# tgialoimtr/cnn_lstm_ctc_ocr

Measured on AMD Instinct MI355X. Metric: line-crops/sec (train step) at 32x256 bs=256; CER vs ref, higher is better.
Workload: dtype bf16

## Files before the change

cnn_lstm_ctc_ocr_amd/csrc/common.h:

```cpp
#pragma once
#include <hip/hip_runtime.h>
#include <cstdint>
#include <cstddef>
#include <mutex>
#include "ocrk.h"

typedef __bf16 bf16;

namespace ocrk {

void set_error(const char* fmt, ...);
int launch_status(const char* what);

inline hipStream_t as_stream(void* s) { return reinterpret_cast<hipStream_t>(s); }

inline int64_t cdiv(int64_t a, int64_t b) { return (a + b - 1) / b; }

constexpr int kMaxDevices = 64;
constexpr int kMaxCuWords = 32;
inline int current_device() {
    int d = 0;
    (void)hipGetDevice(&d);
    return d < 0 ? 0 : (d >= kMaxDevices ? kMaxDevices - 1 : d);
}
// ... 26 lines not shown
    OPT_CONV_ROWS,
    OPT_CONV_ROWS_WIDE,
    OPT_CONV_WGRAD_BLOCKS,
    OPT_LSTM_SPIN_LIMIT,
    OPT_PERSIST_LATE,
    OPT_LSTM_BWD_KSPLIT,
    OPT_LSTM_BWD_PB16,
    OPT_LSTM_BWD_R16,
    OPT_CTC_LDS,
    OPT_PP_PERSIST_NK,
    OPT_PP_DEEP,
    OPT_NT_F32_EXACT,
    OPT_NT_F32_MASK,
    OPT_NT_F32_X6,
    OPT_BEAM_WAVE,
    OPT_BN_BWD_BLOCKS,
    OPT_BN_ROUTE,
    OPT_BN_ROUTE_SEG,
    OPT_BN_ROUTE_NCH,
    OPT_CONV_TN_ITEMS,
    OPT_CONV_TN4_ITEMS,
    OPT_CONV_WGRAD_CUS,
    OPT_F32_MFMA,
    OPT_GEMM_NT,
    OPT_GEMM_NT_STAGED,
    OPT_GEMM_PP,
    OPT_GEMM_PPTN,
    OPT_PP_MIN_N,
    OPT_GEMM_TN,
    OPT_LSTM_DMA,
    OPT_LSTM_BWD_DMA,
    OPT_LSTM_FWD_R16,
    OPT_NT_TAP_UNIFORM,
    OPT_COUNT
};
int64_t opt(Option o);

}

#define OCRK_REQUIRE(cond, ...)                       \
    do {                                                \
        if (!(cond)) {                                  \
            ocrk::set_error(__VA_ARGS__);               \
            return OCRK_ERR_INVALID_ARG;                \
        }                                               \
    } while (0)

__device__ __forceinline__ float to_f32(float x) { return x; }
__device__ __forceinline__ float to_f32(bf16 x) { return (float)x; }
template <typename T> __device__ __forceinline__ T from_f32(float x);
template <> __device__ __forceinline__ float from_f32<float>(float x) { return x; }
template <> __device__ __forceinline__ bf16 from_f32<bf16>(float x) { return (bf16)x; }

__device__ __forceinline__ float sigmoidf_(float x) { return 1.0f / (1.0f + expf(-x)); }

struct F8 { float v[8]; };

template <typename T> __device__ __forceinline__ F8 load8(const T* p);
template <> __device__ __forceinline__ F8 load8<float>(const float* p) {
    F8 r;
    float4 a = reinterpret_cast<const float4*>(p)[0], b = reinterpret_cast<const float4*>(p)[1];
    r.v[0] = a.x; r.v[1] = a.y; r.v[2] = a.z; r.v[3] = a.w;
    r.v[4] = b.x; r.v[5] = b.y; r.v[6] = b.z; r.v[7] = b.w;
    return r;
}
template <> __device__ __forceinline__ F8 load8<bf16>(const bf16* p) {
    union { uint4 q; bf16 e[8]; } u;
    u.q = *reinterpret_cast<const uint4*>(p);
    F8 r;
// ... 94 lines not shown
```

cnn_lstm_ctc_ocr_amd/csrc/gemm.h:

```cpp
#pragma once
#include "common.h"

namespace ocrk {

enum AMode { A_ROWK = 0, A_COLK = 1, A_IM2COL = 2, A_IM2COL_FLIP = 3, A_IM2COL_T = 4 };
enum BMode { B_NK = 0, B_KN = 1 };

struct GemmParams {
    int M, N, K;
    int batch;
    const void* A; int64_t lda; int64_t strideA;
    const void* B; int64_t ldb; int64_t strideB;
    void* C; int64_t ldc; int64_t strideC;
    int c_bf16;
    const float* bias; int64_t strideBias;
    const void* mask; int64_t ldmask;
    int accumulate;
    int relu;
    float alpha;
    float* stats;
    float* splitk_ws;
    int splits;
    int k_chunk;
    int convH, convW, convC;
    int epi_staged;
    const void* mask_bits;
    void* relu_bits;
};

struct TileIdx { int bm, bn; bool valid; };
__device__ __forceinline__ TileIdx xcd_tile(int tm, int tn) {
    const int nT = tm * tn, per = (nT + 7) >> 3;
    const int t = (int)(blockIdx.x & 7) * per + (int)(blockIdx.x >> 3);
    if (t >= nT) return {0, 0, false};
    constexpr int GM = 4;
    const int gsz = GM * tn, grp = t / gsz, first = grp * GM;
    const int gm = min(GM, tm - first), w = t - grp * gsz;
    return {first + w % gm, w / gm, true};
}
__host__ __forceinline__ unsigned xcd_grid(int tm, int tn) { return 8u * (unsigned)((tm * tn + 7) / 8); }

int gemm(const GemmParams& p, int amode, int bmode, int dtype, hipStream_t stream);

size_t gemm_splitk_ws_bytes(int M, int N, int batch, int splits);
int splitk_finish(const GemmParams& p, hipStream_t stream);

int gemm_nt(const GemmParams& p, int amode, int bmode, int dtype, hipStream_t stream);
bool f32_exact_mfma();

int gemm_pp(const GemmParams& p, int amode, int bmode, int dtype, hipStream_t stream);

bool gemm_pptn_covers(int amode, int M, int N, int convC);
int gemm_pptn(const GemmParams& p, int amode, int bmode, int dtype, hipStream_t stream);

int gemm_tn(const GemmParams& p, int amode, int bmode, int dtype, hipStream_t stream);

}
```

cnn_lstm_ctc_ocr_amd/csrc/gemm.hip:

```cpp
#include <atomic>
#include <cstdlib>
#include <type_traits>

#include "gemm.h"
#include "mfma_util.h"

namespace ocrk {

template <int AM, typename CT>
__device__ __forceinline__ const CT* a_addr(const GemmParams& p, const CT* A, int m, int k, bool& ok) {
    if constexpr (AM == A_ROWK) {
        ok = m < p.M && k < p.K;
        return A + (int64_t)m * p.lda + k;
    } else if constexpr (AM == A_COLK) {
        ok = m < p.M && k < p.K;
        return A + (int64_t)k * p.lda + m;
    } else {
        int pix, kidx;
        if constexpr (AM == A_IM2COL_T) { pix = k; kidx = m; ok = k < p.K && m < p.M; }
        else { pix = m; kidx = k; ok = m < p.M && k < p.K; }
        const int C = p.convC, W = p.convW, H = p.convH;
        int tap = kidx / C, c = kidx - tap * C;
        int kh = tap / 3, kw = tap - kh * 3;
        int w = pix % W, t2 = pix / W, h = t2 % H, b = t2 / H;
// ... 498 lines not shown
}

template <typename CT>
static int dispatch_modes(const GemmParams& p, int amode, int bmode, hipStream_t s) {
#define GM(AMx, BMx) if (amode == AMx && bmode == BMx) return launch_tiles<CT, AMx, BMx>(p, s)
    GM(A_ROWK, B_NK);
    GM(A_ROWK, B_KN);
    GM(A_COLK, B_KN);
    GM(A_IM2COL, B_NK);
    GM(A_IM2COL_FLIP, B_NK);
    GM(A_IM2COL_T, B_KN);
#undef GM
    set_error("gemm: unsupported operand modes A=%d B=%d", amode, bmode);
    return OCRK_ERR_INVALID_ARG;
}

int gemm(const GemmParams& p, int amode, int bmode, int dtype, hipStream_t stream) {
    if (p.M <= 0 || p.N <= 0 || p.batch <= 0) return OCRK_OK;
    OCRK_REQUIRE(p.K >= 0 && p.splits >= 1 && p.k_chunk > 0 && p.k_chunk % 32 == 0,
                 "gemm: bad K=%d splits=%d k_chunk=%d", p.K, p.splits, p.k_chunk);
    bool a_rows = (amode == A_COLK || amode == A_IM2COL_T);
    OCRK_REQUIRE(p.K % 8 == 0 || (a_rows && bmode == B_KN),
                 "gemm: K=%d must be a multiple of 8 for k-contiguous operands", p.K);
    OCRK_REQUIRE(!a_rows || p.M % 8 == 0, "gemm: M=%d must be a multiple of 8 for this A mode", p.M);
    OCRK_REQUIRE(bmode != B_KN || p.N % 8 == 0, "gemm: N=%d must be a multiple of 8 for B_KN", p.N);
    OCRK_REQUIRE(amode < A_IM2COL || p.convC % 8 == 0, "gemm: conv channels must be a multiple of 8");
    OCRK_REQUIRE(!(p.stats && (p.splits > 1 || p.batch > 1)), "gemm: stats need splits=1, batch=1");
    OCRK_REQUIRE(!(p.accumulate && p.c_bf16), "gemm: accumulate needs an f32 C");
    if (p.mask_bits || p.relu_bits) {
        const int st = gemm_nt(p, amode, bmode, dtype, stream);
        OCRK_REQUIRE(st >= 0, "gemm: ReLU bit masks need the NT engine (bf16 C, staged epilogue) for this shape");
        return st;
    }
    int nt = gemm_pp(p, amode, bmode, dtype, stream);
    if (nt >= 0) return nt != OCRK_OK ? nt : splitk_finish(p, stream);
    nt = gemm_nt(p, amode, bmode, dtype, stream);
    if (nt < 0) nt = gemm_pptn(p, amode, bmode, dtype, stream);
    if (nt < 0) nt = gemm_tn(p, amode, bmode, dtype, stream);
    if (nt >= 0) return nt != OCRK_OK ? nt : splitk_finish(p, stream);
    if (dtype == OCRK_BF16) return dispatch_modes<bf16>(p, amode, bmode, stream);
    if (dtype == OCRK_F32) return dispatch_modes<float>(p, amode, bmode, stream);
    set_error("gemm: unsupported dtype %d", dtype);
    return OCRK_ERR_INVALID_ARG;
}

}

extern "C" int ocrk_set_f32_gemm_mode(int mode) {
    OCRK_REQUIRE(mode == 0 || mode == 1, "ocrk_set_f32_gemm_mode: mode %d not 0 (bf16x3) or 1 (exact)", mode);
    return ocrk::g_f32_mode.exchange(mode);
}

extern "C" int ocrk_f32_gemm_exact(void) { return ocrk::f32_exact_mfma() ? 1 : 0; }

extern "C" size_t ocrk_gemm_workspace_size(int M, int N, int batch, int splits) {
    return ocrk::gemm_splitk_ws_bytes(M, N, batch, splits);
}

extern "C" int ocrk_gemm(int trans_a, int trans_b, int M, int N, int K, float alpha, const void* A,
                         int64_t lda, int64_t stride_a, const void* B, int64_t ldb, int64_t stride_b,
                         void* C, int64_t ldc, int64_t stride_c, int c_dtype, const float* bias,
                         int relu, int accumulate, int batch, int dtype, int splits, void* ws,
                         size_t ws_bytes, void* stream) {
    ocrk::GemmParams p = {};
    p.M = M; p.N = N; p.K = K; p.batch = batch < 1 ? 1 : batch;
    p.A = A; p.lda = lda; p.strideA = stride_a;
    p.B = B; p.ldb = ldb; p.strideB = stride_b;
    p.C = C; p.ldc = ldc; p.strideC = stride_c;
    p.c_bf16 = c_dtype == OCRK_BF16;
// ... 14 lines not shown
```

cnn_lstm_ctc_ocr_amd/csrc/gemm_pp.hip:

```cpp
#include "gemm.h"
#include "mfma_util.h"

namespace ocrk {

namespace {

constexpr unsigned PP_OOB = 0x80000000u;

__device__ __forceinline__ void pp_dma16(__amdgpu_buffer_rsrc_t r, void* lds, unsigned voff) {
    __builtin_amdgcn_raw_ptr_buffer_load_lds(r, (__attribute__((address_space(3))) void*)lds, 16, voff, 0, 0, 0);
}

__device__ __forceinline__ void pp_barrier() {
    asm volatile("" ::: "memory");
    __builtin_amdgcn_s_barrier();
    asm volatile("" ::: "memory");
}

template <int N> __device__ __forceinline__ void vm_wait_nop() {}

typedef unsigned short u16x4 __attribute__((ext_vector_type(4)));

struct PPItem { int m0, n0, zb, zs; };
__device__ __forceinline__ PPItem pp_item(int w, int tm, int tn, int splits, int BM, int BN) {
    const int nT = tm * tn;
    const int z = w / nT, t = w - z * nT;
    constexpr int GM = 4;
    const int gsz = GM * tn, grp = t / gsz, first = grp * GM;
    const int gm = min(GM, tm - first), r = t - grp * gsz;
    PPItem it;
    it.m0 = (first + r % gm) * BM;
    it.n0 = (r / gm) * BN;
    it.zb = z / splits;
    it.zs = z - it.zb * splits;
    return it;
}

template <int AM, int BN, bool STATS, bool MASK>
__global__ void __launch_bounds__(512) gemm_pp_kernel(const GemmParams p) {
    constexpr int BM = 256, BK = 64, ROWB = 128;
    constexpr int WCOLS = BN / 4;
    constexpr int QN = WCOLS / 32;
    constexpr int A_BYTES = BM * ROWB, BUF = (BM + BN) * ROWB;
    constexpr int NUA = 2;
    constexpr int NUB = BN / 128;
    constexpr int HBLK = WCOLS / 16;
    constexpr int NU0 = NUA, NU1 = NUB, NU2 = NUB, NU3 = NUA;
    constexpr int PITCH = WCOLS * 2 + 16, CPRW = WCOLS / 8;
    constexpr int CR = BN == 256 ? 32 : 64;
    constexpr int NST = 128 * CPRW / 64;
    static_assert(BN == 256 || BN == 128, "BN");
    static_assert(8 * CR * PITCH <= BUF, "staging fits the freed buffer");
    extern __shared__ __attribute__((aligned(16))) char smem[];
    const bf16* mask = reinterpret_cast<const bf16*>(p.mask);

    const int tid = threadIdx.x, lane = tid & 63;
    const int wave = __builtin_amdgcn_readfirstlane(tid >> 6);
    const int wm = wave >> 2, wn = wave & 3;
    const int i16 = lane & 15, g = lane >> 4, sw = lane & 7;

    const int tm = (p.M + BM - 1) / BM, tn = (p.N + BN - 1) / BN;
    const int nitems = tm * tn * p.batch * p.splits;
    const int per = (nitems + 7) >> 3;
    const int xcd = blockIdx.x & 7, slot = blockIdx.x >> 3, sp = gridDim.x >> 3;
    const int wend = min(nitems, (xcd + 1) * per);
    int w_issue = xcd * per + slot;
    if (w_issue >= wend) return;

    const int lrow = lane >> 3;
// ... 287 lines not shown
                    for (int j = 0; j < 2 * QN; ++j) {
                        u16x4 o;
#pragma unroll
                        for (int r = 0; r < 4; ++r)
                            o[r] = __builtin_bit_cast(unsigned short, (bf16)acc[h * (CR / 16) + i][j][r]);
                        *reinterpret_cast<u16x4*>(stg + (i * 16 + i16) * PITCH + (j * 16 + 4 * g) * 2) = o;
                    }
                __builtin_amdgcn_wave_barrier();
#pragma unroll
                for (int q = 0; q < CR * CPRW / 64; ++q) {
                    const int r = r0 + q * (64 / CPRW);
                    const int m = cur_it.m0 + wm * 128 + h * CR + r;
                    const u32x4 v = *reinterpret_cast<const u32x4*>(stg + r * PITCH + c8 * 16);
                    const unsigned off = (m < p.M && n < p.N) ? (unsigned)(((int64_t)m * p.ldc + n) * 2) : PP_OOB;
                    __builtin_amdgcn_raw_buffer_store_b128(v, rc, off, 0, 0);
                }
                __builtin_amdgcn_wave_barrier();
            }
        }
        asm volatile("s_waitcnt lgkmcnt(0)" ::: "memory");
        pp_barrier();
        w_comp += sp;
        if (w_comp >= wend) break;
        cur_it = pp_item(w_comp, tm, tn, p.splits, BM, BN);
        c_nk = max(1, (min(p.K, cur_it.zs * p.k_chunk + p.k_chunk) - cur_it.zs * p.k_chunk + BK - 1) / BK);
        c_kt = 0;
        after_epi = true;
#pragma unroll
        for (int i = 0; i < 8; ++i)
#pragma unroll
            for (int j = 0; j < 2 * QN; ++j) acc[i][j] = floatx4{0.f, 0.f, 0.f, 0.f};
        if (wm == 1) pp_barrier();
    }
}

__device__ __forceinline__ void vm_wait_n(int n) {
    n = __builtin_amdgcn_readfirstlane(n);
    n = n > 63 ? 63 : n;
    switch (n) {
#define VW1(i) case i: vm_wait<i>(); break;
#define VW8(b) VW1(b) VW1(b + 1) VW1(b + 2) VW1(b + 3) VW1(b + 4) VW1(b + 5) VW1(b + 6) VW1(b + 7)
        VW8(0) VW8(8) VW8(16) VW8(24) VW8(32) VW8(40) VW8(48) VW8(56)
#undef VW8
#undef VW1
    default: vm_wait<0>();
    }
}

template <int FAST>
__device__ __forceinline__ void vm_wait_fast(int n) {
    n = __builtin_amdgcn_readfirstlane(n);
    if (n == FAST) vm_wait<FAST>();
    else vm_wait_n(n);
}

template <int BN>
__global__ void __launch_bounds__(512) gemm_pp_deep_kernel(const GemmParams p) {
    constexpr int BM = 256, BK = 64, ROWB = 128;
    constexpr int WCOLS = BN / 4;
    constexpr int QN = WCOLS / 32;
    constexpr int A_BYTES = BM * ROWB, BUF = (BM + BN) * ROWB;
    constexpr int NUA = 2, NUB = BN / 128;
    constexpr int HBLK = WCOLS / 16;
    constexpr int PITCH = WCOLS * 2 + 16, CPRW = WCOLS / 8;
    constexpr int CR = 16;
    constexpr int NST = 128 * CPRW / 64;
    static_assert(BN == 256 || BN == 128, "BN");
    static_assert(CR * PITCH <= (BN == 256 ? 4096 : 2048), "a wave's staging fits its slot piece");
    extern __shared__ __attribute__((aligned(16))) char smem[];

    const int tid = threadIdx.x, lane = tid & 63;
    const int wave = __builtin_amdgcn_readfirstlane(tid >> 6);
    const int wm = wave >> 2, wn = wave & 3;
    const int i16 = lane & 15, g = lane >> 4, sw = lane & 7;

    const int tm = (p.M + BM - 1) / BM, tn = (p.N + BN - 1) / BN;
    const int nitems = tm * tn * p.batch * p.splits;
    const int per = (nitems + 7) >> 3;
    const int xcd = blockIdx.x & 7, slot = blockIdx.x >> 3, sp = gridDim.x >> 3;
    const int wend = min(nitems, (xcd + 1) * per);
    int w_issue = xcd * per + slot;
    if (w_issue >= wend) return;

    const int lrow = lane >> 3;
    const int cs = (lane & 7) ^ lrow;
    int arow[4];
// ... 319 lines not shown
```

cnn_lstm_ctc_ocr_amd/csrc/mfma_util.h:

```cpp
#pragma once
#include "common.h"

namespace ocrk {

typedef __bf16 bf16x8 __attribute__((ext_vector_type(8)));
typedef float floatx4 __attribute__((ext_vector_type(4)));

typedef unsigned int u32x4 __attribute__((ext_vector_type(4)));
typedef float f32x4 __attribute__((ext_vector_type(4)));

template <typename CT> struct V8;
template <> struct V8<bf16> {
    u32x4 q;
    __device__ __forceinline__ unsigned short e(int i) const {
        return (unsigned short)(q[i >> 1] >> (16 * (i & 1)));
    }
};
template <> struct V8<float> {
    f32x4 q0, q1;
    __device__ __forceinline__ float e(int i) const { return i < 4 ? q0[i] : q1[i - 4]; }
};
template <typename CT> struct RawT;
template <> struct RawT<bf16> { using T = unsigned short; };
template <> struct RawT<float> { using T = float; };
// ... 65 lines not shown
    split3_bf16(x.q0[0], x.q0[1], h[0], m[0], l[0]);
    split3_bf16(x.q0[2], x.q0[3], h[1], m[1], l[1]);
    split3_bf16(x.q1[0], x.q1[1], h[2], m[2], l[2]);
    split3_bf16(x.q1[2], x.q1[3], h[3], m[3], l[3]);
    hi = u32x4{h[0], h[1], h[2], h[3]};
    mid = u32x4{m[0], m[1], m[2], m[3]};
    lo = u32x4{l[0], l[1], l[2], l[3]};
}

__device__ __forceinline__ __amdgpu_buffer_rsrc_t uniform_rsrc(const void* base, int64_t bytes) {
    const uint64_t b = (uint64_t)base;
    const unsigned lo = __builtin_amdgcn_readfirstlane((unsigned)b);
    const unsigned hi = __builtin_amdgcn_readfirstlane((unsigned)(b >> 32));
    const int nb = __builtin_amdgcn_readfirstlane(bytes > 0x7fffffff ? 0x7fffffff : (int)bytes);
    return __builtin_amdgcn_make_buffer_rsrc((void*)(((uint64_t)hi << 32) | lo), 0, nb, 0x00020000);
}

typedef int i32x4_t __attribute__((ext_vector_type(4)));
__device__ __forceinline__ i32x4_t uniform_rsrc_words(const void* base, int64_t bytes) {
    const uint64_t b = (uint64_t)base;
    const int lo = (int)__builtin_amdgcn_readfirstlane((unsigned)b);
    const int hi = (int)__builtin_amdgcn_readfirstlane((unsigned)(b >> 32) & 0xffffu);
    const int nb = __builtin_amdgcn_readfirstlane(bytes > 0x7fffffff ? 0x7fffffff : (int)bytes);
    return i32x4_t{lo, hi, nb, 0x00020000};
}

__device__ __forceinline__ void lds_dma16_asm(const i32x4_t& r, void* lds, unsigned voff) {
    const unsigned a = __builtin_amdgcn_readfirstlane(
        (unsigned)(uintptr_t)(__attribute__((address_space(3))) char*)lds);
    asm volatile("s_nop 0\n\tbuffer_load_dwordx4 %0, %1, 0 offen lds"
                 :: "v"(voff), "s"(r), "{m0}"(a) : "memory");
}

}
```

cnn_lstm_ctc_ocr_amd/csrc/runtime.hip:

```cpp
#include <atomic>
#include <cstdarg>
#include <cstdlib>
#include <cstdio>
#include <cstring>
#include <mutex>
#include "common.h"

namespace ocrk {

static thread_local char g_err[1024] = "";

void set_error(const char* fmt, ...) {
    va_list ap;
    va_start(ap, fmt);
    vsnprintf(g_err, sizeof(g_err), fmt, ap);
    va_end(ap);
}

int launch_status(const char* what) {
    hipError_t e = hipGetLastError();
    if (e != hipSuccess) {
        set_error("%s: %s", what, hipGetErrorString(e));
        return OCRK_ERR_HIP;
    }
    return OCRK_OK;
}

namespace {
struct OptDef {
    const char* name;
    int64_t def;
    bool exp = false;
};
constexpr OptDef kOptDefs[OPT_COUNT] = {
    {"CONV_DIRECT", 1}, {"CONV_ROWS", 1}, {"CONV_ROWS_WIDE", 1}, {"CONV_WGRAD_BLOCKS", 1},
    {"LSTM_SPIN_LIMIT", 0}, {"PERSIST_LATE", 1}, {"LSTM_BWD_KSPLIT", 0, true}, {"LSTM_BWD_PB16", 0, true},
    {"LSTM_BWD_R16", 1}, {"CTC_LDS", 1}, {"PP_PERSIST_NK", 8}, {"PP_DEEP", 0, true}, {"NT_F32_EXACT", 1},
    {"NT_F32_MASK", 1},
    {"NT_F32_X6", 0}, {"BEAM_WAVE", 1}, {"BN_BWD_BLOCKS", 2048}, {"BN_ROUTE", 1}, {"BN_ROUTE_SEG", 8}, {"BN_ROUTE_NCH", 4},
    {"CONV_TN_ITEMS", 192},
    {"CONV_TN4_ITEMS", 512}, {"CONV_WGRAD_CUS", 192}, {"F32_MFMA", 0}, {"GEMM_NT", 1}, {"GEMM_NT_STAGED", 1},
    {"GEMM_PP", 1}, {"GEMM_PPTN", 1}, {"PP_MIN_N", 512}, {"GEMM_TN", 1}, {"LSTM_DMA", 1}, {"LSTM_BWD_DMA", 1},
    {"LSTM_FWD_R16", 1}, {"NT_TAP_UNIFORM", 1},
};
std::atomic<int64_t> g_opts[OPT_COUNT];
std::once_flag g_opts_once;

#ifdef OCRK_EXPERIMENTS
constexpr bool kExperiments = true;
#else
constexpr bool kExperiments = false;
#endif

void init_opts() {
    for (int i = 0; i < OPT_COUNT; ++i) {
        if (kOptDefs[i].exp && !kExperiments) {
            g_opts[i].store(kOptDefs[i].def, std::memory_order_relaxed);
            continue;
        }
        char env[64];
        snprintf(env, sizeof(env), "OCRK_%s", kOptDefs[i].name);
        const char* e = getenv(env);
        g_opts[i].store(e && *e ? atoll(e) : kOptDefs[i].def, std::memory_order_relaxed);
    }
}

int find_opt(const char* name) {
    if (!name) return -1;
    if (!strncmp(name, "OCRK_", 5)) name += 5;
    for (int i = 0; i < OPT_COUNT; ++i)
        if (!strcmp(name, kOptDefs[i].name)) return kOptDefs[i].exp && !kExperiments ? -1 : i;
    return -1;
}
}

int64_t opt(Option o) {
    std::call_once(g_opts_once, init_opts);
    return g_opts[o].load(std::memory_order_relaxed);
}

}

extern "C" {

int ocrk_version(void) { return OCRK_ABI_VERSION; }

int ocrk_set_option(const char* name, int64_t value, int64_t* prev) {
    const int i = ocrk::find_opt(name);
    OCRK_REQUIRE(i >= 0, "ocrk_set_option: unknown option '%s'", name ? name : "(null)");
    ocrk::opt((ocrk::Option)i);
    const int64_t old = ocrk::g_opts[i].exchange(value, std::memory_order_relaxed);
    if (prev) *prev = old;
    return OCRK_OK;
}

int ocrk_get_option(const char* name, int64_t* value) {
    const int i = ocrk::find_opt(name);
    OCRK_REQUIRE(i >= 0 && value, "ocrk_get_option: unknown option '%s' or null slot", name ? name : "(null)");
    *value = ocrk::opt((ocrk::Option)i);
    return OCRK_OK;
}

const char* ocrk_last_error(void) { return ocrk::g_err; }

int ocrk_timer_create(void** ev) {
    OCRK_REQUIRE(ev != nullptr, "ocrk_timer_create: null handle slot");
    hipEvent_t e = nullptr;
    if (hipEventCreate(&e) != hipSuccess) return ocrk::launch_status("ocrk_timer_create");
    *ev = e;
    return OCRK_OK;
}
// ... 148 lines not shown
```

cnn_lstm_ctc_ocr_amd/options.py:

```python
import contextlib
import os

_HOST_DEFAULTS = {
    "LSTM_PERSISTENT": 1,
    "F32_TRAIN_EXACT": 0,
    "SIDE_STREAM": 1,
    "CONV_SIDE": 1,
    "CONV12_FUSED": 1,
    "RELU_BITS": 1,
    "POOLED_BN": 1,
    "CONV1_FUSED": 1,
    "CONV12_BWD": 1,
    "TN_ITEMS": 256,
    "TN_ITEMS_L1": 160,
}
KERNEL_OPTIONS = ("CONV_DIRECT", "CONV_ROWS", "CONV_ROWS_WIDE", "CONV_WGRAD_BLOCKS", "LSTM_SPIN_LIMIT",
                  "PERSIST_LATE", "LSTM_BWD_R16", "CTC_LDS",
                  "PP_PERSIST_NK", "NT_F32_EXACT", "NT_F32_MASK",
                  "NT_F32_X6", "BEAM_WAVE", "BN_BWD_BLOCKS", "BN_ROUTE", "BN_ROUTE_SEG", "BN_ROUTE_NCH", "CONV_TN_ITEMS", "CONV_TN4_ITEMS",
                  "CONV_WGRAD_CUS", "F32_MFMA", "GEMM_NT", "GEMM_NT_STAGED", "GEMM_PP", "GEMM_PPTN", "PP_MIN_N", "GEMM_TN",
                  "LSTM_DMA", "LSTM_BWD_DMA", "LSTM_FWD_R16", "NT_TAP_UNIFORM")


def _env_int(name, default):
    v = os.environ.get("OCRK_" + name)
    if v is None or v == "":
        return default
    try:
        return int(v)
    except ValueError:
        raise ValueError(f"OCRK_{name}={v!r}: an integer is expected") from None


_HOST = {k: _env_int(k, d) for k, d in _HOST_DEFAULTS.items()}


def get(name):
    if name in _HOST:
        return _HOST[name]
    if name in KERNEL_OPTIONS:
        import ctypes

        from . import _lib
        v = ctypes.c_int64()
        _lib.call("ocrk_get_option", name.encode(), ctypes.byref(v))
        return v.value
    raise KeyError(f"unknown option {name!r}")


def set(name, value):
    value = int(value)
    if name in _HOST:
        prev, _HOST[name] = _HOST[name], value
        return prev
# ... 21 lines not shown
```

Measured before the change: 53600.

## Add 4-wave 256x256 bf16 GEMM kernels for NK and TN paths

Adds two new large-tile bf16 MFMA GEMM kernels. One is persistent, with 256x256 tiles, 4 waves, LDS DMA double buffering and a fused bias/relu bf16 epilogue, and serves A_ROWK x B_NK. The other handles A_COLK x B_KN with fp32 output and split-k. Both are tried before the existing pp and pptn engines when shapes qualify, and aim for more data reuse per tile and better MFMA/DMA overlap. In exchange they need large LDS use and heavy register pressure from the 8x8 accumulator tiles, add launch-counter bookkeeping, and carry a risk of poor occupancy or tail imbalance on mid-sized shapes.

```diff
diff --git a/cnn_lstm_ctc_ocr_amd/csrc/common.h b/cnn_lstm_ctc_ocr_amd/csrc/common.h
--- a/cnn_lstm_ctc_ocr_amd/csrc/common.h
+++ b/cnn_lstm_ctc_ocr_amd/csrc/common.h
@@ -82,9 +82,12 @@
     OPT_LSTM_BWD_DMA,
     OPT_LSTM_FWD_R16,
     OPT_NT_TAP_UNIFORM,
+    OPT_GEMM_W4,
+    OPT_GEMM_W4_LAUNCHES,
     OPT_COUNT
 };
 int64_t opt(Option o);
+void opt_add(Option o, int64_t d);
 
 }
 
diff --git a/cnn_lstm_ctc_ocr_amd/csrc/gemm.h b/cnn_lstm_ctc_ocr_amd/csrc/gemm.h
--- a/cnn_lstm_ctc_ocr_amd/csrc/gemm.h
+++ b/cnn_lstm_ctc_ocr_amd/csrc/gemm.h
@@ -50,6 +50,9 @@
 
 int gemm_pp(const GemmParams& p, int amode, int bmode, int dtype, hipStream_t stream);
 
+int gemm_w4(const GemmParams& p, int amode, int bmode, int dtype, hipStream_t stream);
+int gemm_w4tn(const GemmParams& p, int amode, int bmode, int dtype, hipStream_t stream);
+
 bool gemm_pptn_covers(int amode, int M, int N, int convC);
 int gemm_pptn(const GemmParams& p, int amode, int bmode, int dtype, hipStream_t stream);
 
diff --git a/cnn_lstm_ctc_ocr_amd/csrc/gemm.hip b/cnn_lstm_ctc_ocr_amd/csrc/gemm.hip
--- a/cnn_lstm_ctc_ocr_amd/csrc/gemm.hip
+++ b/cnn_lstm_ctc_ocr_amd/csrc/gemm.hip
@@ -554,9 +554,11 @@
         OCRK_REQUIRE(st >= 0, "gemm: ReLU bit masks need the NT engine (bf16 C, staged epilogue) for this shape");
         return st;
     }
-    int nt = gemm_pp(p, amode, bmode, dtype, stream);
+    int nt = gemm_w4(p, amode, bmode, dtype, stream);
+    if (nt < 0) nt = gemm_pp(p, amode, bmode, dtype, stream);
     if (nt >= 0) return nt != OCRK_OK ? nt : splitk_finish(p, stream);
     nt = gemm_nt(p, amode, bmode, dtype, stream);
+    if (nt < 0) nt = gemm_w4tn(p, amode, bmode, dtype, stream);
     if (nt < 0) nt = gemm_pptn(p, amode, bmode, dtype, stream);
     if (nt < 0) nt = gemm_tn(p, amode, bmode, dtype, stream);
     if (nt >= 0) return nt != OCRK_OK ? nt : splitk_finish(p, stream);
diff --git a/cnn_lstm_ctc_ocr_amd/csrc/gemm_pp.hip b/cnn_lstm_ctc_ocr_amd/csrc/gemm_pp.hip
--- a/cnn_lstm_ctc_ocr_amd/csrc/gemm_pp.hip
+++ b/cnn_lstm_ctc_ocr_amd/csrc/gemm_pp.hip
@@ -20,21 +20,6 @@
 template <int N> __device__ __forceinline__ void vm_wait_nop() {}
 
 typedef unsigned short u16x4 __attribute__((ext_vector_type(4)));
-
-struct PPItem { int m0, n0, zb, zs; };
-__device__ __forceinline__ PPItem pp_item(int w, int tm, int tn, int splits, int BM, int BN) {
-    const int nT = tm * tn;
-    const int z = w / nT, t = w - z * nT;
-    constexpr int GM = 4;
-    const int gsz = GM * tn, grp = t / gsz, first = grp * GM;
-    const int gm = min(GM, tm - first), r = t - grp * gsz;
-    PPItem it;
-    it.m0 = (first + r % gm) * BM;
-    it.n0 = (r / gm) * BN;
-    it.zb = z / splits;
-    it.zs = z - it.zb * splits;
-    return it;
-}
 
 template <int AM, int BN, bool STATS, bool MASK>
 __global__ void __launch_bounds__(512) gemm_pp_kernel(const GemmParams p) {
@@ -388,26 +373,6 @@
             for (int j = 0; j < 2 * QN; ++j) acc[i][j] = floatx4{0.f, 0.f, 0.f, 0.f};
         if (wm == 1) pp_barrier();
     }
-}
-
-__device__ __forceinline__ void vm_wait_n(int n) {
-    n = __builtin_amdgcn_readfirstlane(n);
-    n = n > 63 ? 63 : n;
-    switch (n) {
-#define VW1(i) case i: vm_wait<i>(); break;
-#define VW8(b) VW1(b) VW1(b + 1) VW1(b + 2) VW1(b + 3) VW1(b + 4) VW1(b + 5) VW1(b + 6) VW1(b + 7)
-        VW8(0) VW8(8) VW8(16) VW8(24) VW8(32) VW8(40) VW8(48) VW8(56)
-#undef VW8
-#undef VW1
-    default: vm_wait<0>();
-    }
-}
-
-template <int FAST>
-__device__ __forceinline__ void vm_wait_fast(int n) {
-    n = __builtin_amdgcn_readfirstlane(n);
-    if (n == FAST) vm_wait<FAST>();
-    else vm_wait_n(n);
 }
 
 template <int BN>
diff --git a/cnn_lstm_ctc_ocr_amd/csrc/gemm_w4.hip b/cnn_lstm_ctc_ocr_amd/csrc/gemm_w4.hip
--- /dev/null
+++ b/cnn_lstm_ctc_ocr_amd/csrc/gemm_w4.hip
@@ -0,0 +1,326 @@
+#include "gemm.h"
+#include "mfma_util.h"
+
+namespace ocrk {
+
+namespace {
+
+constexpr unsigned W4_OOB = 0x80000000u;
+
+__device__ __forceinline__ void w4_barrier() {
+    __builtin_amdgcn_sched_barrier(0);
+    asm volatile("" ::: "memory");
+    __builtin_amdgcn_s_barrier();
+    asm volatile("" ::: "memory");
+    __builtin_amdgcn_sched_barrier(0);
+}
+
+template <int NR, int NM, int REST>
+__device__ __forceinline__ void w4_interleave() {
+#pragma unroll
+    for (int r = 0; r < NR; ++r) {
+        __builtin_amdgcn_sched_group_barrier(0x8, NM, 0);
+        __builtin_amdgcn_sched_group_barrier(0x100, 1, 0);
+    }
+    __builtin_amdgcn_sched_group_barrier(0x8, REST, 0);
+}
+
+typedef unsigned short u16x4 __attribute__((ext_vector_type(4)));
+
+__device__ __forceinline__ i32x4_t w4_rsrc(const void* base, int bytes) {
+    const uint64_t b = (uint64_t)base;
+    return i32x4_t{(int)(unsigned)b, (int)((unsigned)(b >> 32) & 0xffffu), bytes, 0x00020000};
+}
+
+__device__ __forceinline__ void w4_dma16(const i32x4_t& r, unsigned lds, unsigned voff, unsigned soff) {
+    asm volatile("s_nop 0\n\tbuffer_load_dwordx4 %0, %1, %2 offen lds"
+                 :: "v"(voff), "s"(r), "s"(soff), "{m0}"(lds) : "memory");
+}
+
+__global__ void __launch_bounds__(256) gemm_w4_kernel(const GemmParams p) {
+    constexpr int BM = 256, BN = 256, BK = 64, ROWB = 128;
+    constexpr int A_BYTES = BM * ROWB, BUF = (BM + BN) * ROWB;
+    constexpr int NU = 8;
+    constexpr int BIAS_OFF = 2 * BUF, STG_OFF = BIAS_OFF + 4 * 1024;
+    constexpr int PITCH = 128 * 2 + 16, STG = 16 * PITCH;
+    constexpr int NST = 8 * 4;
+    extern __shared__ __attribute__((aligned(16))) char smem[];
+
+    const int tid = threadIdx.x, lane = tid & 63;
+    const int wave = __builtin_amdgcn_readfirstlane(tid >> 6);
+    const int wm = wave >> 1, wn = wave & 1;
+    const int i16 = lane & 15, g = lane >> 4, sw = lane & 7;
+
+    const int tm = (p.M + BM - 1) / BM, tn = (p.N + BN - 1) / BN;
+    const int nitems = tm * tn * p.batch;
+    const int per = (nitems + 7) >> 3;
+    const int xcd = blockIdx.x & 7, slot = blockIdx.x >> 3, sp = gridDim.x >> 3;
+    const int wend = min(nitems, (xcd + 1) * per);
+    int w_issue = xcd * per + slot;
+    if (w_issue >= wend) return;
+
+    typedef const __attribute__((address_space(4))) GemmParams* KArgs;
+    const bool has_bias = p.bias != nullptr;
+    const int c_nk = max(1, (p.K + BK - 1) / BK);
+
+    const int lrow = lane >> 3;
+    const int cs = (lane & 7) ^ lrow;
+    i32x4_t ra, rb;
+    int i_m0 = 0, i_n0 = 0, i_zb = 0, i_kt = 0, i_cnt = 0;
+    const unsigned a_lane = (unsigned)(lrow * p.lda * 2), b_lane = (unsigned)(lrow * p.ldb * 2);
+    auto setup_issue = [&](int w) {
+        const PPItem it = pp_item(w, tm, tn, 1, BM, BN);
+        ra = w4_rsrc(reinterpret_cast<const bf16*>(p.A) + it.zb * p.strideA, p.M * (int)p.lda * 2);
+        rb = w4_rsrc(reinterpret_cast<const bf16*>(p.B) + it.zb * p.strideB, p.N * (int)p.ldb * 2);
+        i_m0 = it.m0;
+        i_n0 = it.n0;
+        i_zb = it.zb;
+        i_kt = 0;
+    };
+    int ops = 0;
+    const unsigned lds0 = (unsigned)(uintptr_t)(__attribute__((address_space(3))) char*)smem;
+    auto lane_off = [&](unsigned lane_row, bool on) -> unsigned {
+        const int k = i_kt * BK + 8 * cs;
+        return on && k < p.K ? lane_row + (unsigned)(k * 2) : W4_OOB;
+    };
+    auto unit_base = [&](int first, unsigned buf, int& row, unsigned& lds) {
+        row = first + wave * 8;
+        lds = buf + wave * 8 * ROWB;
+        asm volatile("" : "+s"(row), "+s"(lds));
+    };
+    auto dma_a = [&](int i, int row, unsigned lds, unsigned va) {
+        const int mrow = row + i * 32;
+        const unsigned soff = mrow < p.M ? (unsigned)(mrow * (int)p.lda * 2) : 0u;
+        w4_dma16(ra, lds + i * 32 * ROWB, lrow < p.M - mrow ? va : W4_OOB, soff);
+    };
+    auto dma_b = [&](int i, int row, unsigned lds, unsigned vb) {
+        const int ncol = row + i * 32;
+        const unsigned soff = ncol < p.N ? (unsigned)(ncol * (int)p.ldb * 2) : 0u;
+        w4_dma16(rb, lds + i * 32 * ROWB, lrow < p.N - ncol ? vb : W4_OOB, soff);
+    };
+    auto dma_bias = [&](bool on) {
+        if (i_kt == 0 && has_bias && wave == 0) {
+            const int n = i_n0 + 4 * lane;
+            KArgs e = (KArgs)__builtin_amdgcn_kernarg_segment_ptr();
+            asm volatile("" : "+s"(e));
+            const i32x4_t rbias = w4_rsrc(e->bias + i_zb * e->strideBias, p.N * 4);
+            w4_dma16(rbias, lds0 + BIAS_OFF + (i_cnt & 3) * 1024, on && n < p.N ? (unsigned)(n * 4) : W4_OOB, 0u);
+            ops += 1;
+        }
+    };
+    auto advance_issue = [&]() -> bool {
+        if (++i_kt < c_nk) return true;
+        w_issue += sp;
+        ++i_cnt;
+        if (w_issue >= wend) return false;
+        setup_issue(w_issue);
+        return true;
+    };
+
+    int w_comp = w_issue, c_cnt = 0;
+
+    bf16x8 af0[8], bf0[8], af1[8], bf1[8];
+    const int a_base = (wm * 128 + i16) * ROWB, b_base = A_BYTES + (wn * 128 + i16) * ROWB;
+    auto read_a = [&](const char* buf, int kk, bf16x8 (&fr)[8]) {
+#pragma unroll
+        for (int i = 0; i < 8; ++i)
+            fr[i] = *reinterpret_cast<const bf16x8*>(buf + a_base + i * 16 * ROWB + (((kk * 4 + g) ^ sw) << 4));
+    };
+    auto read_b = [&](const char* buf, int kk, bf16x8 (&fr)[8]) {
+#pragma unroll
+        for (int j = 0; j < 8; ++j)
+            fr[j] = *reinterpret_cast<const bf16x8*>(buf + b_base + j * 16 * ROWB + (((kk * 4 + g) ^ sw) << 4));
+    };
+    floatx4 acc[8][8];
+    auto zero_acc = [&]() {
+#pragma unroll
+        for (int i = 0; i < 8; ++i)
+#pragma unroll
+            for (int j = 0; j < 8; ++j) acc[i][j] = floatx4{0.f, 0.f, 0.f, 0.f};
+    };
+    auto mfma_rows = [&](auto I0_, const bf16x8 (&a)[8], const bf16x8 (&b)[8]) {
+        constexpr int I0 = decltype(I0_)::value;
+#pragma unroll
+        for (int i = I0; i < I0 + 4; ++i)
+#pragma unroll
+            for (int j = 0; j < 8; ++j)
+                acc[i][j] = __builtin_amdgcn_mfma_f32_16x16x32_bf16(b[j], a[i], acc[i][j], 0, 0, 0);
+    };
+    using R0 = std::integral_constant<int, 0>;
+    using R4 = std::integral_constant<int, 4>;
+    (void)read_b;
+
+    int mA1 = 0, mB1 = 0, mA2 = 0, mB2 = 0;
+    setup_issue(w_issue);
+    bool more = true;
+    int m0done = 0;
+#pragma unroll
+    for (int t = 0; t < 2; ++t) {
+        const unsigned va = lane_off(a_lane, more), vb = lane_off(b_lane, more);
+        int row;
+        unsigned lds;
+        unit_base(i_m0, lds0 + t * BUF, row, lds);
+#pragma unroll
+        for (int i = 0; i < NU; ++i) dma_a(i, row, lds, va);
+        ops += NU;
+        mA1 = ops;
+        dma_bias(more);
+        unit_base(i_n0, lds0 + t * BUF + A_BYTES, row, lds);
+#pragma unroll
+        for (int i = 0; i < NU; ++i) dma_b(i, row, lds, vb);
+        ops += NU;
+        mB1 = ops;
+        if (t == 0) m0done = ops;
+        if (more) more = advance_issue();
+    }
+    vm_wait_n(ops - m0done);
+    w4_barrier();
+    read_a(smem, 0, af0);
+    read_b(smem, 0, bf0);
+
+    int s = 0;
+    for (;;) {
+      zero_acc();
+      for (int c_kt = 0; c_kt < c_nk; ++c_kt) {
+        char* cur = smem + (s & 1) * BUF;
+        const char* nxt = smem + ((s + 1) & 1) * BUF;
+        __builtin_amdgcn_sched_barrier(0);
+        __builtin_amdgcn_s_setprio(1);
+        read_a(cur, 1, af1);
+        read_b(cur, 1, bf1);
+        mfma_rows(R0{}, af0, bf0);
+        mfma_rows(R4{}, af0, bf0);
+        w4_interleave<16, 3, 16>();
+        __builtin_amdgcn_s_setprio(0);
+        __builtin_amdgcn_sched_barrier(0);
+        asm volatile("s_waitcnt lgkmcnt(0)" ::: "memory");
+        vm_wait_fast<NU>(ops - mA1);
+        w4_barrier();
+        {
+            const unsigned va = lane_off(a_lane, more);
+            int row;
+            unsigned lds;
+            unit_base(i_m0, lds0 + (s & 1) * BUF, row, lds);
+            __builtin_amdgcn_s_setprio(1);
+#pragma unroll
+            for (int q = 0; q < 8; ++q) {
+                af0[q] = *reinterpret_cast<const bf16x8*>(nxt + a_base + q * 16 * ROWB + ((g ^ sw) << 4));
+#pragma unroll
+                for (int j = (q & 1) * 4; j < (q & 1) * 4 + 4; ++j)
+                    acc[q >> 1][j] = __builtin_amdgcn_mfma_f32_16x16x32_bf16(bf1[j], af1[q >> 1], acc[q >> 1][j], 0, 0, 0);
+                dma_a(q, row, lds, va);
+                __builtin_amdgcn_sched_barrier(0);
+            }
+            __builtin_amdgcn_s_setprio(0);
+            ops += NU;
+            mA2 = ops;
+        }
+        vm_wait_fast<NU>(ops - mB1);
+        w4_barrier();
+        {
+            const unsigned vb = lane_off(b_lane, more);
+            dma_bias(more);
+            int row;
+            unsigned lds;
+            unit_base(i_n0, lds0 + (s & 1) * BUF + A_BYTES, row, lds);
+            __builtin_amdgcn_s_setprio(1);
+#pragma unroll
+            for (int q = 0; q < 8; ++q) {
+                bf0[q] = *reinterpret_cast<const bf16x8*>(nxt + b_base + q * 16 * ROWB + ((g ^ sw) << 4));
+#pragma unroll
+                for (int j = (q & 1) * 4; j < (q & 1) * 4 + 4; ++j)
+                    acc[4 + (q >> 1)][j] =
+                        __builtin_amdgcn_mfma_f32_16x16x32_bf16(bf1[j], af1[4 + (q >> 1)], acc[4 + (q >> 1)][j], 0, 0, 0);
+                dma_b(q, row, lds, vb);
+                __builtin_amdgcn_sched_barrier(0);
+            }
+            __builtin_amdgcn_s_setprio(0);
+            ops += NU;
+            mB2 = ops;
+        }
+        if (more) more = advance_issue();
+        mA1 = mA2;
+        mB1 = mB2;
+        ++s;
+      }
+
+        {
+            int el;
+            asm volatile("v_mbcnt_lo_u32_b32 %0, -1, 0\n\tv_mbcnt_hi_u32_b32 %0, -1, %0" : "=v"(el));
+            const PPItem cur_it = pp_item(w_comp, tm, tn, 1, BM, BN);
+            KArgs e = (KArgs)__builtin_amdgcn_kernarg_segment_ptr();
+            asm volatile("" : "+s"(e));
+            const int i16 = el & 15, g = el >> 4;
+            const char* bslot = smem + BIAS_OFF + (c_cnt & 3) * 1024 + (wn * 128 + 4 * g) * 4;
+            floatx4 bv[8];
+#pragma unroll
+            for (int j = 0; j < 8; ++j) {
+                bv[j] = floatx4{0.f, 0.f, 0.f, 0.f};
+                if (has_bias) bv[j] = *reinterpret_cast<const floatx4*>(bslot + j * 64);
+            }
+            char* stg = smem + STG_OFF + wave * STG;
+            bf16* Cb = reinterpret_cast<bf16*>(e->C) + cur_it.zb * e->strideC;
+            const __amdgpu_buffer_rsrc_t rc =
+                __builtin_amdgcn_make_buffer_rsrc(Cb, 0, ((p.M - 1) * (int)e->ldc + p.N) * 2, 0x00020000);
+            const int c8 = el & 15, r0 = el >> 4;
+            const int n = cur_it.n0 + wn * 128 + 8 * c8;
+#pragma unroll
+            for (int h = 0; h < 8; ++h) {
+#pragma unroll
+                for (int j = 0; j < 8; ++j) {
+                    floatx4 v = acc[h][j] * e->alpha + bv[j];
+                    if (e->relu) {
+#pragma unroll
+                        for (int r = 0; r < 4; ++r) v[r] = fmaxf(v[r], 0.f);
+                    }
+                    u16x4 o;
+#pragma unroll
+                    for (int r = 0; r < 4; ++r) o[r] = __builtin_bit_cast(unsigned short, (bf16)v[r]);
+                    *reinterpret_cast<u16x4*>(stg + i16 * PITCH + (j * 16 + 4 * g) * 2) = o;
+                }
+                __builtin_amdgcn_wave_barrier();
+#pragma unroll
+                for (int q = 0; q < 4; ++q) {
+                    const int r = r0 + q * 4;
+                    const int m = cur_it.m0 + wm * 128 + h * 16 + r;
+                    const u32x4 v = *reinterpret_cast<const u32x4*>(stg + r * PITCH + c8 * 16);
+                    const unsigned off = (m < p.M && n < p.N) ? (unsigned)(((int64_t)m * e->ldc + n) * 2) : W4_OOB;
+                    __builtin_amdgcn_raw_buffer_store_b128(v, rc, off, 0, 0);
+                }
+                __builtin_amdgcn_wave_barrier();
+            }
+            ops += NST;
+        }
+        w_comp += sp;
+        ++c_cnt;
+        if (w_comp >= wend) break;
+    }
+    vm_wait<0>();
+}
+
+}
+
+int gemm_w4(const GemmParams& p, int amode, int bmode, int dtype, hipStream_t stream) {
+    const int64_t mode = opt(OPT_GEMM_W4);
+    if (mode == 0 || dtype != OCRK_BF16 || amode != A_ROWK || bmode != B_NK) return -1;
+    if (!p.c_bf16 || p.accumulate || p.splits != 1 || p.mask || p.stats || p.mask_bits || p.relu_bits) return -1;
+    if (p.N % 8 != 0 || p.K % 8 != 0 || (int64_t)p.M < 4096 || p.N < 96) return -1;
+    if ((int64_t)p.M * p.lda * 2 >= (1ll << 31) || (int64_t)p.N * p.ldb * 2 >= (1ll << 31) ||
+        (int64_t)p.M * p.ldc * 2 >= (1ll << 31))
+        return -1;
+    if (p.ldc % 8 != 0 || p.strideC % 8 != 0 || (uintptr_t)p.C % 16 != 0) return -1;
+    if (p.bias && (uintptr_t)p.bias % 16 != 0) return -1;
+    if (p.lda % 8 != 0 || p.ldb % 8 != 0) return -1;
+    if (mode == 1 && (p.K < 2048 || p.N < 512)) return -1;
+    constexpr int LDS = 2 * 512 * 128 + 4 * 1024 + 4 * 16 * (128 * 2 + 16);
+    static DeviceOnce configured;
+    set_dyn_lds(configured, reinterpret_cast<const void*>(&gemm_w4_kernel), LDS);
+    const int ncu = cu_count();
+    const int64_t items = cdiv(p.M, 256) * cdiv(p.N, 256) * (int64_t)p.batch;
+    const int64_t grid = std::min<int64_t>(cdiv(items, 8) * 8, (int64_t)(ncu / 8) * 8);
+    gemm_w4_kernel<<<dim3((unsigned)grid), 256, LDS, stream>>>(p);
+    opt_add(OPT_GEMM_W4_LAUNCHES, 1);
+    return launch_status("gemm_w4");
+}
+
+}
diff --git a/cnn_lstm_ctc_ocr_amd/csrc/gemm_w4tn.hip b/cnn_lstm_ctc_ocr_amd/csrc/gemm_w4tn.hip
--- /dev/null
+++ b/cnn_lstm_ctc_ocr_amd/csrc/gemm_w4tn.hip
@@ -0,0 +1,224 @@
+#include "gemm.h"
+#include "mfma_util.h"
+
+namespace ocrk {
+
+namespace {
+
+constexpr unsigned W4T_OOB = 0x80000000u;
+
+__device__ __forceinline__ void w4t_barrier() {
+    __builtin_amdgcn_sched_barrier(0);
+    asm volatile("" ::: "memory");
+    __builtin_amdgcn_s_barrier();
+    asm volatile("" ::: "memory");
+    __builtin_amdgcn_sched_barrier(0);
+}
+
+__device__ __forceinline__ void w4t_dma16(const i32x4_t& r, unsigned lds, unsigned voff, unsigned soff) {
+    asm volatile("s_nop 0\n\tbuffer_load_dwordx4 %0, %1, %2 offen lds"
+                 :: "v"(voff), "s"(r), "s"(soff), "{m0}"(lds) : "memory");
+}
+
+__global__ void __launch_bounds__(256) gemm_w4tn_kernel(const GemmParams p) {
+    constexpr int BM = 256, BN = 256, BK = 64, ROWB = 128, BLK = BK * ROWB;
+    constexpr int A_BYTES = 4 * BLK, BUF = 8 * BLK;
+    constexpr int NU = 8;
+    extern __shared__ __attribute__((aligned(16))) char smem[];
+
+    const int tid = threadIdx.x, lane = tid & 63;
+    const int wave = __builtin_amdgcn_readfirstlane(tid >> 6);
+    const int wm = wave >> 1, wn = wave & 1;
+    const int i16 = lane & 15, g = lane >> 4;
+
+    const int tm = (p.M + BM - 1) / BM, tn = (p.N + BN - 1) / BN;
+    const int nT = tm * tn;
+    const int nitems = nT * p.batch * p.splits;
+    const int per = (nitems + 7) >> 3;
+    const int w = (int)(blockIdx.x & 7) * per + (int)(blockIdx.x >> 3);
+    if (w >= nitems || (int)(blockIdx.x >> 3) >= per) return;
+    const int z = w / nT, t = w - z * nT;
+    constexpr int GM = 4;
+    const int gsz = GM * tn, grp = t / gsz, first = grp * GM;
+    const int gm = min(GM, tm - first), rr = t - grp * gsz;
+    const int m0 = (first + rr % gm) * BM, n0 = (rr / gm) * BN;
+    const int zb = z / p.splits, zs = z - zb * p.splits;
+    const int kbeg = zs * p.k_chunk;
+    const int kend = min(p.K, kbeg + p.k_chunk);
+    const int nk = max(1, (kend - kbeg + BK - 1) / BK);
+    const uint64_t pa = (uint64_t)(reinterpret_cast<const bf16*>(p.A) + zb * p.strideA);
+    const uint64_t pb = (uint64_t)(reinterpret_cast<const bf16*>(p.B) + zb * p.strideB);
+    const i32x4_t ra = {(int)(unsigned)pa, (int)((unsigned)(pa >> 32) & 0xffffu), p.K * (int)p.lda * 2, 0x00020000};
+    const i32x4_t rb = {(int)(unsigned)pb, (int)((unsigned)(pb >> 32) & 0xffffu), p.K * (int)p.ldb * 2, 0x00020000};
+
+    const int lrow = lane >> 3;
+    const int chunk = (lane & 7) ^ lrow;
+    const unsigned lds0 = (unsigned)(uintptr_t)(__attribute__((address_space(3))) char*)smem;
+    unsigned va[2], vb[2];
+    int krow[2];
+#pragma unroll
+    for (int h = 0; h < 2; ++h) {
+        krow[h] = (h * 4 + wave) * 8 + lrow;
+        va[h] = (unsigned)((krow[h] * (int)p.lda + m0 + 8 * chunk) * 2);
+        vb[h] = (unsigned)((krow[h] * (int)p.ldb + n0 + 8 * chunk) * 2);
+    }
+    auto dma_a = [&](int i, int kt, unsigned buf, bool on) {
+        const int k0 = kbeg + kt * BK;
+        const bool ok = on && k0 + krow[i & 1] < kend && m0 + 64 * (i >> 1) + 8 * chunk < p.M;
+        const unsigned soff = on ? (unsigned)(k0 * (int)p.lda * 2 + 128 * (i >> 1)) : 0u;
+        w4t_dma16(ra, buf + (i >> 1) * BLK + ((i & 1) * 4 + wave) * 1024, ok ? va[i & 1] : W4T_OOB, soff);
+    };
+    auto dma_b = [&](int i, int kt, unsigned buf, bool on) {
+        const int k0 = kbeg + kt * BK;
+        const bool ok = on && k0 + krow[i & 1] < kend && n0 + 64 * (i >> 1) + 8 * chunk < p.N;
+        const unsigned soff = on ? (unsigned)(k0 * (int)p.ldb * 2 + 128 * (i >> 1)) : 0u;
+        w4t_dma16(rb, buf + A_BYTES + (i >> 1) * BLK + ((i & 1) * 4 + wave) * 1024, ok ? vb[i & 1] : W4T_OOB, soff);
+    };
+
+    const int kr0 = 4 * g + (i16 >> 2), cq = 4 * (i16 & 3);
+    auto tr_off = [&](int blk, int col, int kk) {
+        const int r = kk * 32 + kr0;
+        return blk * BLK + r * ROWB + ((((col >> 3) ^ (r & 7))) << 4) + (col & 7) * 2;
+    };
+    auto frag_a = [&](const char* buf, int i, int kk) {
+        return frag_tr(reinterpret_cast<const unsigned short*>(buf + tr_off(2 * wm + (i >> 2), (i & 3) * 16 + cq, kk)),
+                       16 * (ROWB / 2));
+    };
+    auto frag_b = [&](const char* buf, int j, int kk) {
+        return frag_tr(reinterpret_cast<const unsigned short*>(
+                           buf + A_BYTES + tr_off(2 * wn + (j >> 2), (j & 3) * 16 + cq, kk)),
+                       16 * (ROWB / 2));
+    };
+
+    floatx4 acc[8][8];
+#pragma unroll
+    for (int i = 0; i < 8; ++i)
+#pragma unroll
+        for (int j = 0; j < 8; ++j) acc[i][j] = floatx4{0.f, 0.f, 0.f, 0.f};
+    bf16x8 af0[8], bf0[8], af1[8], bf1[8];
+
+#pragma unroll
+    for (int t2 = 0; t2 < 2; ++t2) {
+#pragma unroll
+        for (int i = 0; i < NU; ++i) dma_a(i, t2, lds0 + t2 * BUF, t2 < nk);
+#pragma unroll
+        for (int i = 0; i < NU; ++i) dma_b(i, t2, lds0 + t2 * BUF, t2 < nk);
+    }
+    vm_wait<2 * NU>();
+    w4t_barrier();
+#pragma unroll
+    for (int i = 0; i < 8; ++i) af0[i] = frag_a(smem, i, 0);
+#pragma unroll
+    for (int j = 0; j < 8; ++j) bf0[j] = frag_b(smem, j, 0);
+
+    for (int kt = 0; kt < nk; ++kt) {
+        const char* cur = smem + (kt & 1) * BUF;
+        const char* nxt = smem + ((kt + 1) & 1) * BUF;
+        const unsigned curl = lds0 + (kt & 1) * BUF;
+        const bool more = kt + 2 < nk;
+        __builtin_amdgcn_sched_barrier(0);
+        __builtin_amdgcn_s_setprio(1);
+#pragma unroll
+        for (int i = 0; i < 8; ++i) af1[i] = frag_a(cur, i, 1);
+#pragma unroll
+        for (int j = 0; j < 8; ++j) bf1[j] = frag_b(cur, j, 1);
+#pragma unroll
+        for (int i = 0; i < 8; ++i)
+#pragma unroll
+            for (int j = 0; j < 8; ++j)
+                acc[i][j] = __builtin_amdgcn_mfma_f32_16x16x32_bf16(bf0[j], af0[i], acc[i][j], 0, 0, 0);
+#pragma unroll
+        for (int r = 0; r < 24; ++r) {
+            __builtin_amdgcn_sched_group_barrier(0x8, 2, 0);
+            __builtin_amdgcn_sched_group_barrier(0x100, 1, 0);
+        }
+#pragma unroll
+        for (int r = 0; r < 8; ++r) {
+            __builtin_amdgcn_sched_group_barrier(0x8, 1, 0);
+            __builtin_amdgcn_sched_group_barrier(0x100, 1, 0);
+        }
+        __builtin_amdgcn_sched_group_barrier(0x8, 8, 0);
+        __builtin_amdgcn_s_setprio(0);
+        __builtin_amdgcn_sched_barrier(0);
+        asm volatile("s_waitcnt lgkmcnt(0)" ::: "memory");
+        vm_wait<NU>();
+        w4t_barrier();
+        __builtin_amdgcn_s_setprio(1);
+#pragma unroll
+        for (int q = 0; q < 8; ++q) {
+            af0[q] = frag_a(nxt, q, 0);
+#pragma unroll
+            for (int j = (q & 1) * 4; j < (q & 1) * 4 + 4; ++j)
+                acc[q >> 1][j] = __builtin_amdgcn_mfma_f32_16x16x32_bf16(bf1[j], af1[q >> 1], acc[q >> 1][j], 0, 0, 0);
+            dma_a(q, kt + 2, curl, more);
+            __builtin_amdgcn_sched_barrier(0);
+        }
+        __builtin_amdgcn_s_setprio(0);
+        vm_wait<NU>();
+        w4t_barrier();
+        __builtin_amdgcn_s_setprio(1);
+#pragma unroll
+        for (int q = 0; q < 8; ++q) {
+            bf0[q] = frag_b(nxt, q, 0);
+#pragma unroll
+            for (int j = (q & 1) * 4; j < (q & 1) * 4 + 4; ++j)
+                acc[4 + (q >> 1)][j] =
+                    __builtin_amdgcn_mfma_f32_16x16x32_bf16(bf1[j], af1[4 + (q >> 1)], acc[4 + (q >> 1)][j], 0, 0, 0);
+            dma_b(q, kt + 2, curl, more);
+            __builtin_amdgcn_sched_barrier(0);
+        }
+        __builtin_amdgcn_s_setprio(0);
+        __builtin_amdgcn_sched_barrier(0);
+    }
+    vm_wait<0>();
+
+    const int mrow0 = m0 + wm * 128 + i16, ncol0 = n0 + wn * 128 + 4 * g;
+    float* C;
+    int64_t ldc;
+    bool acc_c;
+    if (p.splits > 1) {
+        C = p.splitk_ws + ((int64_t)zb * p.splits + zs) * (int64_t)p.M * p.N;
+        ldc = p.N;
+        acc_c = false;
+    } else {
+        C = reinterpret_cast<float*>(p.C) + zb * p.strideC;
+        ldc = p.ldc;
+        acc_c = p.accumulate != 0;
+    }
+#pragma unroll
+    for (int i = 0; i < 8; ++i) {
+        const int m = mrow0 + i * 16;
+        if (m >= p.M) continue;
+#pragma unroll
+        for (int j = 0; j < 8; ++j) {
+            const int n = ncol0 + j * 16;
+            if (n >= p.N) continue;
+            floatx4* dst = reinterpret_cast<floatx4*>(C + (int64_t)m * ldc + n);
+            floatx4 v = acc[i][j] * p.alpha;
+            if (acc_c) v += *dst;
+            *dst = v;
+        }
+    }
+}
+
+}
+
+int gemm_w4tn(const GemmParams& p, int amode, int bmode, int dtype, hipStream_t stream) {
+    const int64_t mode = opt(OPT_GEMM_W4);
+    if (mode == 0 || dtype != OCRK_BF16 || amode != A_COLK || bmode != B_KN) return -1;
+    if (!gemm_pptn_covers(amode, p.M, p.N, p.convC)) return -1;
+    if (p.c_bf16 || p.bias || p.relu || p.mask || p.stats) return -1;
+    if (p.ldb % 8 != 0 || p.lda % 8 != 0) return -1;
+    if (p.splits == 1 && (p.ldc % 4 != 0 || (uintptr_t)p.C % 16 != 0 || p.strideC % 4 != 0)) return -1;
+    if (p.splits > 1 && (uintptr_t)p.splitk_ws % 16 != 0) return -1;
+    if ((int64_t)p.K * p.lda * 2 >= (1ll << 31) || (int64_t)p.K * p.ldb * 2 >= (1ll << 31)) return -1;
+    constexpr int LDS = 2 * 8 * 64 * 128;
+    static DeviceOnce configured;
+    set_dyn_lds(configured, reinterpret_cast<const void*>(&gemm_w4tn_kernel), LDS);
+    const int64_t items = cdiv(p.M, 256) * cdiv(p.N, 256) * (int64_t)p.batch * p.splits;
+    gemm_w4tn_kernel<<<dim3((unsigned)(cdiv(items, 8) * 8)), 256, LDS, stream>>>(p);
+    opt_add(OPT_GEMM_W4_LAUNCHES, 1);
+    return launch_status("gemm_w4tn");
+}
+
+}
diff --git a/cnn_lstm_ctc_ocr_amd/csrc/mfma_util.h b/cnn_lstm_ctc_ocr_amd/csrc/mfma_util.h
--- a/cnn_lstm_ctc_ocr_amd/csrc/mfma_util.h
+++ b/cnn_lstm_ctc_ocr_amd/csrc/mfma_util.h
@@ -121,4 +121,40 @@
                  :: "v"(voff), "s"(r), "{m0}"(a) : "memory");
 }
 
+
+struct PPItem { int m0, n0, zb, zs; };
+__device__ __forceinline__ PPItem pp_item(int w, int tm, int tn, int splits, int BM, int BN) {
+    const int nT = tm * tn;
+    const int z = w / nT, t = w - z * nT;
+    constexpr int GM = 4;
+    const int gsz = GM * tn, grp = t / gsz, first = grp * GM;
+    const int gm = min(GM, tm - first), r = t - grp * gsz;
+    PPItem it;
+    it.m0 = (first + r % gm) * BM;
+    it.n0 = (r / gm) * BN;
+    it.zb = z / splits;
+    it.zs = z - it.zb * splits;
+    return it;
 }
+
+__device__ __forceinline__ void vm_wait_n(int n) {
+    n = __builtin_amdgcn_readfirstlane(n);
+    n = n > 63 ? 63 : n;
+    switch (n) {
+#define VW1(i) case i: vm_wait<i>(); break;
+#define VW8(b) VW1(b) VW1(b + 1) VW1(b + 2) VW1(b + 3) VW1(b + 4) VW1(b + 5) VW1(b + 6) VW1(b + 7)
+        VW8(0) VW8(8) VW8(16) VW8(24) VW8(32) VW8(40) VW8(48) VW8(56)
+#undef VW8
+#undef VW1
+    default: vm_wait<0>();
+    }
+}
+
+template <int FAST>
+__device__ __forceinline__ void vm_wait_fast(int n) {
+    n = __builtin_amdgcn_readfirstlane(n);
+    if (n == FAST) vm_wait<FAST>();
+    else vm_wait_n(n);
+}
+
+}
diff --git a/cnn_lstm_ctc_ocr_amd/csrc/runtime.hip b/cnn_lstm_ctc_ocr_amd/csrc/runtime.hip
--- a/cnn_lstm_ctc_ocr_amd/csrc/runtime.hip
+++ b/cnn_lstm_ctc_ocr_amd/csrc/runtime.hip
@@ -41,7 +41,7 @@
     {"CONV_TN_ITEMS", 192},
     {"CONV_TN4_ITEMS", 512}, {"CONV_WGRAD_CUS", 192}, {"F32_MFMA", 0}, {"GEMM_NT", 1}, {"GEMM_NT_STAGED", 1},
     {"GEMM_PP", 1}, {"GEMM_PPTN", 1}, {"PP_MIN_N", 512}, {"GEMM_TN", 1}, {"LSTM_DMA", 1}, {"LSTM_BWD_DMA", 1},
-    {"LSTM_FWD_R16", 1}, {"NT_TAP_UNIFORM", 1},
+    {"LSTM_FWD_R16", 1}, {"NT_TAP_UNIFORM", 1}, {"GEMM_W4", 1}, {"GEMM_W4_LAUNCHES", 0},
 };
 std::atomic<int64_t> g_opts[OPT_COUNT];
 std::once_flag g_opts_once;
@@ -77,6 +77,11 @@
 int64_t opt(Option o) {
     std::call_once(g_opts_once, init_opts);
     return g_opts[o].load(std::memory_order_relaxed);
+}
+
+void opt_add(Option o, int64_t d) {
+    std::call_once(g_opts_once, init_opts);
+    g_opts[o].fetch_add(d, std::memory_order_relaxed);
 }
 
 }
diff --git a/cnn_lstm_ctc_ocr_amd/options.py b/cnn_lstm_ctc_ocr_amd/options.py
--- a/cnn_lstm_ctc_ocr_amd/options.py
+++ b/cnn_lstm_ctc_ocr_amd/options.py
@@ -19,7 +19,8 @@
                   "PP_PERSIST_NK", "NT_F32_EXACT", "NT_F32_MASK",
                   "NT_F32_X6", "BEAM_WAVE", "BN_BWD_BLOCKS", "BN_ROUTE", "BN_ROUTE_SEG", "BN_ROUTE_NCH", "CONV_TN_ITEMS", "CONV_TN4_ITEMS",
                   "CONV_WGRAD_CUS", "F32_MFMA", "GEMM_NT", "GEMM_NT_STAGED", "GEMM_PP", "GEMM_PPTN", "PP_MIN_N", "GEMM_TN",
-                  "LSTM_DMA", "LSTM_BWD_DMA", "LSTM_FWD_R16", "NT_TAP_UNIFORM")
+                  "LSTM_DMA", "LSTM_BWD_DMA", "LSTM_FWD_R16", "NT_TAP_UNIFORM",
+                  "GEMM_W4", "GEMM_W4_LAUNCHES")
 
 
 def _env_int(name, default):
```

Result: faster. 54570 (median of 6 runs) (+1.8%).
